# NethermindEth/starkpack-winterfell

Hardware: AMD Instinct MI355X
Metric: trace-LDE + Merkle-commit field-ops/s (wall-clock ms in ms_per_step), 2^20x8 f64 trace blowup=8 (higher is better)
Workload: dtype u64 (Goldilocks, Montgomery form) + u32 (BLAKE3)

## Files before the change

### include/wf_lde.h

```cpp
#ifndef WF_LDE_H
#define WF_LDE_H

#include <stddef.h>
#include <stdint.h>

#ifdef __cplusplus
extern "C" {
#endif

typedef struct wf_ctx wf_ctx;

enum wf_field { WF_FIELD_F64 = 1, WF_FIELD_F128 = 2 };
enum wf_hasher {
    WF_HASH_BLAKE3 = 0,
    WF_HASH_SHA3_256 = 1,
    WF_HASH_RP64_256 = 16,
    WF_HASH_RPJIVE64_256 = 18,
    WF_HASH_GRIFFINJIVE64_256 = 20
};

enum wf_status {
    WF_OK = 0,
    WF_ERR_FIELD = -10,
    WF_ERR_EXTENSION = -11,
// ... 18 lines not shown
    uint32_t log2_blowup;
    uint32_t n_cols;
    uint32_t n_traces;
    uint32_t digest_bytes;
    uint32_t hasher;
    uint8_t domain_offset[16];
} wf_params;


int wf_ctx_create(int device, wf_ctx **out);
void wf_ctx_destroy(wf_ctx *ctx);
int wf_ctx_release_cached(wf_ctx *ctx);
int wf_ctx_set_digest_bytes(wf_ctx *ctx, uint32_t digest_bytes);
int wf_ctx_set_hasher(wf_ctx *ctx, uint32_t hasher);
int wf_plan_digits(uint32_t field, uint32_t log2_n, uint32_t n_segments, uint32_t digits_out[4]);
const char *wf_last_error(void);
int wf_device_count(void);
int wf_ctx_synchronize(wf_ctx *ctx);
void *wf_ctx_stream(wf_ctx *ctx);

int wf_ctx_profile_enable(wf_ctx *ctx, int on);
int wf_ctx_profile_read(wf_ctx *ctx, int max_entries, const char **names, float *ms);

int wf_params_check(const wf_params *p, int is_constraint);

size_t wf_elem_bytes(uint32_t field);
size_t wf_row_width(const wf_params *p);
size_t wf_column_bytes(const wf_params *p);
size_t wf_lde_bytes(const wf_params *p);
size_t wf_digests_bytes(const wf_params *p);
// ... 214 lines not shown
```

### starkpack-winterfell_amd/capi.py

```python
from __future__ import annotations

import ctypes as C
import os
import weakref

import numpy as np

from .build import lib_path

F64, F128 = 1, 2
BLAKE3, SHA3_256, RP64_256, RPJIVE64_256, GRIFFINJIVE64_256 = 0, 1, 16, 18, 20
ELEM_WORDS = {F64: 1, F128: 2}

SYMBOLS = [
    "wf_ctx_create", "wf_ctx_destroy", "wf_last_error", "wf_device_count", "wf_ctx_synchronize", "wf_ctx_stream",
    "wf_ctx_release_cached", "wf_ctx_set_digest_bytes", "wf_ctx_set_hasher", "wf_plan_digits", "wf_commitment_query", "wf_ctx_profile_enable", "wf_ctx_profile_read", "wf_params_check", "wf_elem_bytes", "wf_row_width", "wf_column_bytes", "wf_lde_bytes", "wf_digests_bytes",
    "wf_trace_commit", "wf_constraint_commit", "wf_trace_commit_dev", "wf_constraint_commit_dev",
    "wf_trace_commit_shard_dev", "wf_merkle_build_dev", "wf_trace_commit_resident", "wf_trace_commit_resident_async", "wf_commitment_wait", "wf_constraint_commit_resident", "wf_commitment_destroy", "wf_commitment_root",
    "wf_commitment_info", "wf_commitment_read_rows", "wf_commitment_read_lde", "wf_commitment_read_lde_strided", "wf_deep_compose", "wf_commitment_evaluate_polys_at_points", "wf_constraint_commit_from_evaluations", "wf_constraint_commit_from_tables", "wf_commitment_query_many", "wf_commitment_prove", "wf_commitment_prove_batch",
    "wf_evaluate_columns_at", "wf_commitment_evaluate_polys_at", "wf_fri_layer_commit", "wf_fri_apply_drp", "wf_fri_layer_commit_dev", "wf_fri_apply_drp_dev",
    "wf_fri_prover_create", "wf_fri_prover_destroy", "wf_fri_num_layers", "wf_fri_prover_begin", "wf_fri_prover_begin_dev", "wf_fri_prover_begin_poly",
    "wf_fri_prover_commit_layer", "wf_fri_prover_fold", "wf_fri_prover_set_remainder", "wf_fri_prover_num_layers",
    "wf_fri_prover_layer", "wf_fri_prover_reset", "wf_fri_fold_positions",
    "wf_fft_evaluate_poly", "wf_fft_evaluate_poly_with_offset", "wf_fft_interpolate_poly",
    "wf_fft_interpolate_poly_with_offset", "wf_evaluate_polys_over", "wf_hash_rows", "wf_merkle_build", "wf_grind_seeds",
    "wf_comm_unique_id", "wf_comm_create", "wf_comm_create_with_transport", "wf_comm_destroy", "wf_comm_rank",
    "wf_comm_world", "wf_comm_rccl_version", "wf_comm_rccl_path", "wf_comm_stream_wait", "wf_comm_all_gather", "wf_comm_all_gather_roots", "wf_comm_barrier",
    "wf_comm_max_f64", "wf_comm_gather_f64", "wf_comm_info", "wf_shard_proofs", "wf_shard_cosets", "wf_shard_route", "wf_comm_all_gather_leaf_shards",
    "wf_trace_commit_sharded_dev", "wf_trace_commit_sharded_resident", "wf_sharded_commitment_destroy",
    "wf_sharded_commitment_root", "wf_sharded_commitment_query", "wf_sharded_commitment_polys",
    "wf_constraint_evaluate", "wf_evaluations_info", "wf_evaluations_read", "wf_evaluations_destroy",
    "wf_constraint_commit_from_device_tables",
]


class WfError(RuntimeError):
    def __init__(self, code: int, msg: str):
        super().__init__(f"wf_lde error {code}: {msg}")
        self.code = code


class Params(C.Structure):
    _fields_ = [
        ("field", C.c_uint32), ("ext_degree", C.c_uint32), ("log2_trace_len", C.c_uint32),
        ("log2_blowup", C.c_uint32), ("n_cols", C.c_uint32), ("n_traces", C.c_uint32),
        ("digest_bytes", C.c_uint32), ("hasher", C.c_uint32), ("domain_offset", C.c_uint8 * 16),
    ]
# ... 167 lines not shown
        L.wf_fri_prover_reset.argtypes = [vp]
        L.wf_fri_fold_positions.argtypes = [vp, sz, sz, u32, vp, C.POINTER(sz)]
        L.wf_fft_evaluate_poly.argtypes = [vp, u32, u32, vp, sz]
        L.wf_fft_interpolate_poly.argtypes = [vp, u32, u32, vp, sz]
        L.wf_fft_interpolate_poly_with_offset.argtypes = [vp, u32, u32, vp, sz, vp]
        L.wf_fft_evaluate_poly_with_offset.argtypes = [vp, u32, u32, vp, sz, vp, sz, vp]
        L.wf_evaluate_polys_over.argtypes = [vp, PP, vp, vp]
        L.wf_hash_rows.argtypes = [vp, u32, vp, sz, sz, vp]
        L.wf_merkle_build.argtypes = [vp, vp, sz, vp]
        L.wf_grind_seeds.argtypes = [vp, vp, sz, u32, C.c_uint64, C.c_uint64, vp, vp, vp]
        L.wf_device_count.argtypes = []
        L.wf_ctx_release_cached.argtypes = [vp]
        L.wf_ctx_set_digest_bytes.argtypes = [vp, u32]
        L.wf_ctx_set_hasher.argtypes = [vp, u32]
        L.wf_plan_digits.argtypes = [u32, u32, u32, C.POINTER(u32)]
        L.wf_commitment_query.argtypes = [vp, vp, sz, vp, vp, vp, sz, vp, C.POINTER(sz), C.POINTER(sz), C.POINTER(u32)]
        pu32, pu64 = C.POINTER(u32), C.POINTER(C.c_uint64)
        L.wf_comm_unique_id.argtypes = [vp]
        L.wf_comm_create.argtypes = [vp, vp, i32, i32, C.POINTER(vp)]
        L.wf_comm_create_with_transport.argtypes = [vp, C.POINTER(Transport), i32, i32, C.POINTER(vp)]
        L.wf_comm_destroy.argtypes = [vp]
        L.wf_comm_destroy.restype = None
        L.wf_comm_rank.argtypes = [vp]
        L.wf_comm_world.argtypes = [vp]
        L.wf_comm_rccl_version.argtypes = []
        L.wf_trace_commit_resident_async.argtypes = [vp, PP, vp, C.POINTER(vp)]
        L.wf_commitment_wait.argtypes = [vp]
        L.wf_comm_rccl_path.argtypes = []
        L.wf_comm_rccl_path.restype = C.c_char_p
        L.wf_comm_stream_wait.argtypes = [vp, vp]
# ... 573 lines not shown
        vecs, k = [], 0
        for i in range(q.n_vectors):
            vecs.append([bytes(nodes[k + j]) for j in range(int(counts[i]))])
            k += int(counts[i])
        out.append((rows, ([bytes(x) for x in leaves[:len(pos)]], vecs, int(q.depth))))
    return out


def plan_digits(field: int, log2_n: int, n_segments: int = 1):
    out = (C.c_uint32 * 4)()
    n = load().wf_plan_digits(field, log2_n, n_segments, out)
    _check(n if n < 0 else 0)
    return [int(out[i]) for i in range(n)]


def fri_num_layers(folding: int, blowup: int, remainder_max_degree: int, domain_size: int) -> int:
    return int(load().wf_fri_num_layers(folding, blowup, remainder_max_degree, domain_size))


def fri_fold_positions(positions, source_domain_size: int, folding: int) -> np.ndarray:
    pos = np.ascontiguousarray(positions, dtype=np.uint64)
    out = np.empty(max(1, len(pos)), dtype=np.uint64)
    n_out = C.c_size_t()
    _check(load().wf_fri_fold_positions(_p(pos), len(pos), source_domain_size, folding, _p(out), C.byref(n_out)))
    return out[:n_out.value].copy()


class FriProver:

    def __init__(self, ctx: "Context", field, ext, folding, blowup, remainder_max_degree, offset: int):
# ... 61 lines not shown
```

### starkpack-winterfell_amd/csrc/context.hip

```cpp
#include "wf_internal.hpp"

#include <atomic>

#include "field.hpp"
#include "hasher_table.hpp"

using namespace wf;

static thread_local char g_err[512] = "";

std::atomic<uint64_t> g_fail_epoch{0};
uint64_t fail_epoch() { return g_fail_epoch.load(std::memory_order_relaxed); }

int fail(int code, const char *fmt, ...) {
    g_fail_epoch.fetch_add(1, std::memory_order_relaxed);
    va_list ap;
    va_start(ap, fmt);
    vsnprintf(g_err, sizeof(g_err), fmt, ap);
    va_end(ap);
    return code;
}

const char *last_error_text() { return g_err; }

// ... 12 lines not shown
    t.persistent_always = getenv("WF_EXP_PERSISTENT_ALWAYS") != nullptr;
    t.no_persistent = getenv("WF_EXP_NO_PERSISTENT") != nullptr;
    if (const char *e = getenv("WF_EXP_MERKLE_L2_MIN")) {
        const int v = atoi(e);
        if (v >= 10 && v <= 30) t.merkle_l2_min = (uint32_t)v;
    }
    t.no_pipeline = getenv("WF_EXP_NO_PIPELINE") != nullptr;
    t.no_tail_pack = getenv("WF_EXP_NO_TAIL_PACK") != nullptr;
    t.no_coset_inner = getenv("WF_EXP_NO_COSET_INNER") != nullptr;
    t.no_gtab = getenv("WF_EXP_NO_GTAB") != nullptr;
    t.no_staged_chunks = getenv("WF_EXP_NO_STAGED_CHUNKS") != nullptr;
    t.no_gtab1 = getenv("WF_EXP_NO_GTAB1") != nullptr;
    t.no_ftab = getenv("WF_EXP_NO_FTAB") != nullptr;
    t.no_gtab1_wide = getenv("WF_EXP_NO_GTAB1_WIDE") != nullptr;
    t.gtab1_f64 = getenv("WF_EXP_GTAB1_F64") != nullptr;
    if (const char *e = getenv("WF_EXP_WIDE_TI")) {
        const int v = atoi(e);
        if (v == 1 || v == 2 || v == 4 || v == 8) t.wide_ti = (uint32_t)v;
    }
    if (const char *e = getenv("WF_EXP_PIPELINE_MIN_BYTES")) {
        const long long v = atoll(e);
        if (v >= 0 && v <= (1ll << 40)) t.pipeline_min_bytes = (size_t)v;
    }
    if (const char *e = getenv("WF_EXP_FAIL_AFTER_SEGMENT")) {
        const int v = atoi(e);
        if (v >= 0 && v < 4096) t.fail_after_segment = v;
    }
    if (const char *e = getenv("WF_EXP_GRIND_WINDOW_LOG2")) {
        const int v = atoi(e);
        if (v >= 2 && v <= 30) t.grind_window_log2 = (uint32_t)v;
// ... 403 lines not shown
```

### starkpack-winterfell_amd/csrc/path.hip

```cpp
#include "wf_internal.hpp"

#include "kernels.hpp"
#include "keccak_dev.hpp"
#include "keccak_kernels.hpp"
#include "merkle_plan.hpp"
#include "rescue_kernels.hpp"
#include "hasher_dispatch.hpp"
#include "seg_kernels.hpp"
#include "col_kernels.hpp"
#include "fri_kernels.hpp"
#include "tables.hpp"

using namespace wf;

#if defined(WF_EXPERIMENTS) && defined(WF_EXP_STAMPS)
static unsigned long long *g_exp_stamps = nullptr;
static unsigned long long *exp_stamps_buffer() {
    if (!g_exp_stamps && hipMalloc(&g_exp_stamps, 4096 * 8 * 8) == hipSuccess) (void)hipMemset(g_exp_stamps, 0, 4096 * 8 * 8);
    return g_exp_stamps;
}
extern "C" int wf_exp_stamps_read(unsigned long long *out, int clear) {
    if (!g_exp_stamps) return -1;
    if (hipMemcpy(out, g_exp_stamps, 4096 * 8 * 8, hipMemcpyDeviceToHost) != hipSuccess) return -2;
    if (clear) (void)hipMemset(g_exp_stamps, 0, 4096 * 8 * 8);
// ... 188 lines not shown
    T *out;
    uint32_t logN, n_seg, n_cosets;
    bool rows_out;
    void *leaves = nullptr;
    uint32_t hash_epr = 0;
    uint32_t digest_words = 8;
    bool *fused = nullptr;
    const TableSet *pre;
    const T *fin_tab = nullptr;
    bool pad_traces = false;
    bool pad_in_kernel = false;
    uint32_t base_cols, total_base_cols, coset0;
    uint64_t row_width, trace_lde_elems;
    uint32_t seg0 = 0, seg_cnt = 0;
    int phase = 0;
};

template <class F>
static int run_seg_transform(wf_ctx *ctx, hipStream_t st, const SegDesc<F> &d) {
    typedef typename F::T T;
    const bool inverse = !d.rows_out;
    TableSet *tw;
    int rc = root_tables<F>(ctx, d.logN, inverse, &tw);
    if (rc) return rc;
    const Plan plan = seg_plan<F>(d.logN, d.n_seg, ctx->tune.max_digit, ctx->tune.full_tiles);
    const uint64_t N = (uint64_t)1 << d.logN;

    SegArgs<F> a;
    memset(&a, 0, sizeof(a));
    a.logN = d.logN;
    a.n_seg = d.n_seg;
    a.n_cosets = d.n_cosets;
    a.tw = as_pow2l<F>(*tw);
    if (d.pre) {
        a.pre = as_pow2l<F>(*d.pre);
        a.pre_lo_stride = d.pre->lo_stride;
        a.pre_hi_stride = d.pre->hi_stride;
    }
    a.base_cols = d.base_cols;
    a.total_base_cols = d.total_base_cols;
    a.store_cols = d.pad_in_kernel ? d.n_seg * SegCfg<F>::S : d.base_cols;
// ... 520 lines not shown
            rc = run_merkle(ctx, st, d_leaves, Nrows, d_nodes, p->hasher, p->digest_bytes);
            if (rc) return rc;
        }
    }
    prof_mark(ctx, st, "between_calls");
    return 0;
}

template <class F>
static int trace_commit_dev(wf_ctx *ctx, const wf_params *p, const void *d_trace, void *d_polys, void *d_lde,
                            void *d_leaves, void *d_nodes, hipStream_t st, hipEvent_t input_read = nullptr) {
    PathBufs<F> b;
    int rc = path_buffers<F>(ctx, p, b);
    if (rc) return rc;
    const uint64_t R = (uint64_t)1 << p->log2_trace_len;
    rc = run_xpose<F>(ctx, st, true, d_trace, b.segA, R, p->ext_degree, b.total_base_cols, b.n_seg);
    if (rc) return rc;
    if (input_read) HIP_TRY(hipEventRecord(input_read, st));
    SegDesc<F> d;
    memset(&d, 0, sizeof(d));
    d.in = b.segA;
    d.work = b.segA;
    d.out = b.segB;
    d.logN = p->log2_trace_len;
    d.n_seg = b.n_seg;
    d.n_cosets = 1;
    d.rows_out = false;
    rc = run_seg_transform<F>(ctx, st, d);
    if (rc) return rc;
    rc = run_xpose<F>(ctx, st, false, b.segB, d_polys, R, p->ext_degree, b.total_base_cols, b.n_seg);
    if (rc) return rc;
    return evaluate_and_commit<F>(ctx, st, p, b, d_lde, d_leaves, d_nodes);
}

template <class F>
static int trace_commit_pipelined_impl(wf_ctx *ctx, const wf_params *p, const void *const *cols_in, void *d_stage, void *d_polys,
                                       void *d_lde, void *d_leaves, void *d_nodes, hipStream_t st, void *const *polys_out) {
    typedef typename F::T T;
    constexpr uint32_t S = SegCfg<F>::S;
    PathBufs<F> b;
    int rc = path_buffers<F>(ctx, p, b);
    if (rc) return rc;
// ... 2 lines not shown
    if (!ctx->copy_stream) HIP_TRY(hipStreamCreateWithFlags(&ctx->copy_stream, hipStreamNonBlocking));
    while (ctx->seg_events.size() < (size_t)b.n_seg + 1) {
        hipEvent_t e;
        HIP_TRY(hipEventCreateWithFlags(&e, hipEventDisableTiming));
        ctx->seg_events.push_back(e);
    }
    HIP_TRY(hipEventRecord(ctx->seg_events[b.n_seg], st));
    HIP_TRY(hipStreamWaitEvent(ctx->copy_stream, ctx->seg_events[b.n_seg], 0));
    for (uint32_t g = 0; g < b.n_seg; g++) {
        if (ctx->tune.fail_after_segment >= 0 && (int)g == ctx->tune.fail_after_segment)
            return fail(WF_ERR_HIP, "injected failure after %u uploaded segment(s) (WF_EXP_FAIL_AFTER_SEGMENT)", g);
        for (size_t i = (size_t)g * S; i < std::min<size_t>(TC, (size_t)(g + 1) * S); i++)
            HIP_TRY(hipMemcpyAsync((char *)d_stage + i * colb, cols_in[i], colb, hipMemcpyHostToDevice, ctx->copy_stream));
        HIP_TRY(hipEventRecord(ctx->seg_events[g], ctx->copy_stream));
        HIP_TRY(hipStreamWaitEvent(st, ctx->seg_events[g], 0));
        rc = run_xpose<F>(ctx, st, true, d_stage, b.segA, R, 1, b.total_base_cols, b.n_seg, g, 1);
        if (rc) return rc;
        SegDesc<F> d;
        memset(&d, 0, sizeof(d));
        d.in = b.segA + (size_t)g * R * S;
        d.work = (T *)d.in;
        d.out = b.segB + (size_t)g * R * S;
        d.logN = p->log2_trace_len;
        d.n_seg = 1;
        d.n_cosets = 1;
        d.rows_out = false;
        if ((rc = run_seg_transform<F>(ctx, st, d))) return rc;
        if ((rc = evaluate_and_commit<F>(ctx, st, p, b, d_lde, d_leaves, d_nodes, 0, 0, false, 1, g, 1))) return rc;
    }
    if ((rc = run_xpose<F>(ctx, st, false, b.segB, d_polys, R, 1, b.total_base_cols, b.n_seg))) return rc;
    if (polys_out) HIP_TRY(hipEventRecord(ctx->seg_events[b.n_seg], st));
    if ((rc = evaluate_and_commit<F>(ctx, st, p, b, d_lde, d_leaves, d_nodes, 0, 0, false, 2))) return rc;
    if (polys_out) {
        HIP_TRY(hipStreamWaitEvent(ctx->copy_stream, ctx->seg_events[b.n_seg], 0));
        if ((rc = download_columns(ctx, polys_out, d_polys, TC, colb, ctx->copy_stream))) return rc;
        HIP_TRY(hipStreamSynchronize(ctx->copy_stream));
    }
    return 0;
}

template <class F>
// ... 45 lines not shown
    return p->field == WF_FIELD_F64 ? packed_shape<F64>(1, base, base, 1u << p->log2_blowup, &cpr, &lg)
                                    : packed_shape<F128>(1, base, base, 1u << p->log2_blowup, &cpr, &lg);
}

extern "C" {

int wf_plan_digits(uint32_t field, uint32_t log2_n, uint32_t n_segments, uint32_t digits_out[4]) {
    if (!digits_out) return fail(WF_ERR_ARG, "digits_out is null");
    if (field != WF_FIELD_F64 && field != WF_FIELD_F128) return fail(WF_ERR_FIELD, "unknown field id %u", field);
    if (log2_n < 1 || log2_n > 40) return fail(WF_ERR_TRACE_LENGTH, "transform size out of range");
    const Plan p = field == WF_FIELD_F64 ? seg_plan<F64>(log2_n, n_segments) : seg_plan<F128>(log2_n, n_segments);
    for (int i = 0; i < 4; i++) digits_out[i] = i < p.n_pass ? p.dig[i] : 0;
    return p.n_pass;
}


int wf_trace_commit_dev(wf_ctx *ctx, const wf_params *p, const void *d_trace, void *d_polys, void *d_lde,
                        void *d_leaves, void *d_nodes, void *stream) {
    if (!ctx) return fail(WF_ERR_ARG, "ctx is null");
    int rc = check_params(p, false);
    if (rc) return rc;
    if (!d_trace || !d_polys || !d_lde) return fail(WF_ERR_ARG, "null device buffer");
    HIP_TRY(hipSetDevice(ctx->device));
    hipStream_t st = stream ? (hipStream_t)stream : ctx->stream;
    WF_ENTER(ctx, st);
    if (p->field == WF_FIELD_F64) return trace_commit_dev<F64>(ctx, p, d_trace, d_polys, d_lde, d_leaves, d_nodes, st);
    return trace_commit_dev<F128>(ctx, p, d_trace, d_polys, d_lde, d_leaves, d_nodes, st);
}

int wf_constraint_commit_dev(wf_ctx *ctx, const wf_params *p, const void *d_polys, void *d_lde, void *d_leaves,
// ... 481 lines not shown
```

### starkpack-winterfell_amd/csrc/seg_kernels.hpp

```cpp
#pragma once

#include <hip/hip_runtime.h>
#include <stdint.h>

#include "field.hpp"
#include "kernels.hpp"

#ifndef WF_EXPERIMENTS
#undef WF_EXP_SKIP_LOAD
#undef WF_EXP_SKIP_NTT
#undef WF_EXP_SKIP_STORE
#undef WF_EXP_LOCAL_STORE
#undef WF_EXP_STAMPS
#endif

namespace wf {

template <class F>
struct SegCfg {
    static constexpr uint32_t S = 64 / F::BYTES;
    static constexpr uint32_t HP = S / 2;
    static constexpr bool RADIX16 = F::BYTES == 8;
    static constexpr bool RADIX8 = F::BYTES == 16;
    static constexpr uint32_t LOAD_BATCH = F::BYTES == 8 ? 8 : 4;
// ... 25 lines not shown
template <>
__device__ __forceinline__ Pair<uint64_t> pair_from<F64>(const uint4 &qa, const uint4 &) {
    Pair<uint64_t> v;
    v.a = ((uint64_t)qa.y << 32) | qa.x;
    v.b = ((uint64_t)qa.w << 32) | qa.z;
    return v;
}
template <>
__device__ __forceinline__ Pair<U128> pair_from<F128>(const uint4 &qa, const uint4 &qb) {
    Pair<U128> v;
    v.a = U128{((uint64_t)qa.y << 32) | qa.x, ((uint64_t)qa.w << 32) | qa.z};
    v.b = U128{((uint64_t)qb.y << 32) | qb.x, ((uint64_t)qb.w << 32) | qb.z};
    return v;
}

enum : int { SEG_OUT_SEG = 0, SEG_OUT_ROWS = 1 };

template <int LOGD>
__device__ __forceinline__ uint32_t tile_threads() {
    return LOGD ? (1u << (LOGD ? LOGD - 1 : 0)) : blockDim.x;
}
#define WF_TILE_BOUNDS(LOGD, GENERIC) __launch_bounds__((LOGD) ? (1 << ((LOGD) ? (LOGD) - 1 : 0)) : (GENERIC), (LOGD) ? 4 : 1)

__device__ __forceinline__ uint64_t xcd_group_index(uint64_t b, uint64_t total) {
    if ((total & 63) != 0) return b;
    const uint64_t xcd = b & 7, seq = b >> 3;
    return (((seq >> 3) << 3) + xcd) * 8 + (seq & 7);
}

__device__ __forceinline__ uint64_t coset_inner_split(uint64_t bid, uint32_t lc, uint32_t &c) {
    const uint64_t hi = bid >> 6;
// ... 33 lines not shown
    uint32_t tail_pad;
    uint32_t seg_stride;
    uint32_t coset0;
    uint32_t rows_per_k;
    uint32_t cpr_log, lg_log;
    uint64_t row_width;
    uint64_t trace_lde_elems;
    uint32_t *leaves;
    uint32_t hash_epr;
    uint32_t digest_words;
    uint32_t *chunk_cvs;
    uint32_t n_chunks;
    uint32_t *tile_counters;
    const T *src_tail;
    uint32_t tail_cols;
#ifdef WF_EXP_STAMPS
    unsigned long long *stamps;
#endif
};

#if defined(WF_EXPERIMENTS) && defined(WF_EXP_R8_NO_SPLIT)
constexpr uint32_t R8_SPLIT = 0;
#else
constexpr uint32_t R8_SPLIT = 4;
#endif
__host__ __device__ constexpr uint32_t radix8_rounds(uint32_t logD) {
    return (R8_SPLIT == 4 && logD >= 4 && logD % 3 == 1) ? logD / 3 - 1 : logD / 3;
}

template <class F>
// ... 431 lines not shown
    if (logD >= 2) w4 = twd[D >> 2];
    while (cur > 0) {
        if (cur >= 2) {
            seg_round4<F, DIR, false, LANES>(x, twd, w4, logD, cur, nthr, threadIdx.x);
            cur -= 2;
        } else {
            seg_round2<F, LANES>(x, logD, nthr, threadIdx.x);
            cur = 0;
        }
        __syncthreads();
    }
}

template <class F, int EVAL, bool PACKED = false, int LOGD = 0>
__global__ void WF_TILE_BOUNDS(LOGD, 1024) k_seg_strided(SegArgs<F> a) {
    typedef typename F::T T;
    if (LOGD) a.logD = LOGD;
    const uint32_t NT = tile_threads<LOGD>();
    typedef Pair<T> P2;
    constexpr uint32_t S = SegCfg<F>::S, HP = SegCfg<F>::HP;
    constexpr uint32_t hp_shift = HP == 4 ? 2 : 1;
    extern __shared__ __attribute__((aligned(16))) unsigned char smem_raw[];
    const uint32_t D = 1u << a.logD;
    T *x = reinterpret_cast<T *>(smem_raw);
    T *twd = x + (size_t)D * S;
    constexpr bool ONE_TABLE = F::BYTES == 16;
    T *aux = ONE_TABLE ? twd : twd + D;

    uint64_t bid = xcd_group_index(blockIdx.x, gridDim.x);
    const uint32_t logI = ilog2_pow2(a.I), logO = ilog2_pow2(a.O);
// ... 170 lines not shown
#undef WF_FILL_ITEM
    }
    if (!direct || scale_in) __syncthreads();
    if (ONE_TABLE) {
        if (threadIdx.x < D) twd[kq[0]] = unpark<F>(twk0);
        if (threadIdx.x + NT < D) twd[kq[1]] = unpark<F>(twk1);
        __syncthreads();
    } else {
#pragma unroll
        for (uint32_t q = 0; q < 2; q++) {
            const uint32_t k = threadIdx.x + q * NT;
            if (k < D) aux[k] = fo[q];
        }
    }
#ifndef WF_EXP_SKIP_NTT
    seg_lds_ntt<F, EVAL ? 1 : -1, (LOGD ? (1u << LOGD) : 0u)>(x, twd, a.logD, NT, direct ? vr : nullptr, direct);
#else
    if (direct && has16) {
#pragma unroll
        for (uint32_t q = 0; q < 16; q++) x[(q * m16 + j16) * S + l16] = vr[q];
    }
    __syncthreads();
#endif
    if (ONE_TABLE) {
        if (threadIdx.x < D) aux[threadIdx.x] = unpark<F>(fok0);
        if (threadIdx.x + NT < D) aux[threadIdx.x + NT] = unpark<F>(fok1);
        __syncthreads();
    }

    T start_a = F::one(), start_b = F::one();
    if (PACKED && a.pre_on) {
// ... 2 lines not shown
    }
    const uint32_t pstride = NT >> hp_shift, pos0 = threadIdx.x >> hp_shift;
    if (pos0 >= D) return;
    const uint32_t k0 = seg_digit_reverse<F>(pos0, a.logD);
    T *dst_lane = dst + row0 * S + lane_a;
    const uint32_t k_shift = logI + (S == 8 ? 3 : 2);
    for (uint32_t pj = 0; pj < D; pj += pstride) {
        const uint32_t k = k0 | seg_digit_reverse<F>(pj, a.logD);
        P2 v = *reinterpret_cast<P2 *>(x + (pos0 + pj) * S + lane_a);
        const T f = aux[k];
        v.a = F::mul(v.a, f);
        v.b = F::mul(v.b, f);
        if (PACKED && a.pre_on) {
            v.a = F::mul(v.a, start_a);
            v.b = F::mul(v.b, start_b);
        }
#ifdef WF_EXP_SKIP_STORE
        if (*reinterpret_cast<const uint32_t *>(&v.a) == a.logN + 77777u)
#endif
        store_pair(dst_lane + ((uint64_t)k << k_shift), v);
    }
}

template <class F, int EVAL, int TI, int GTAB = 0, int LOGD = 0>
__global__ void __launch_bounds__(1024) k_seg_strided_wide(SegArgs<F> a) {
    if (LOGD) a.logD = LOGD;
    static_assert(SegCfg<F>::RADIX16 && TI >= 2 && (TI & (TI - 1)) == 0, "f64 tiles of 2, 4 or 8 inner positions");
    typedef typename F::T T;
    typedef Pair<T> P2;
    constexpr uint32_t S = SegCfg<F>::S, LANES = TI * S, HPW = LANES / 2;
// ... 177 lines not shown
        for (uint32_t pos = psub; pos < D; pos += pstep) {
            const uint64_t k = rev_o + ((uint64_t)seg_digit_reverse<F>(pos, a.logD) << out_shift);
            const uint64_t off = (uint64_t)(uint32_t)k * k_stride;
            const T v0 = d0 && in0 ? x[pos * S + (b0 - lo)] : F::zero();
            const T v1 = d1 && in1 ? x[pos * S + (b1 - lo)] : F::zero();
            if (in0 && in1)
                store_pair(row + off, Pair<T>{v0, v1});
            else if (in0)
                row[off] = v0;
            else
                row[off + 1] = v1;
        }
    }
}

template <class F, int OUT, bool PACKED = false, int LOGD = 0>
__global__ void WF_TILE_BOUNDS(LOGD, 1024) k_seg_last(SegArgs<F> a) {
    typedef typename F::T T;
    const uint32_t logD_ = LOGD ? (uint32_t)LOGD : a.logD;
    const uint32_t NT = tile_threads<LOGD>();
    typedef Pair<T> P2;
    constexpr uint32_t S = SegCfg<F>::S, HP = SegCfg<F>::HP;
    constexpr uint32_t hp_shift = HP == 4 ? 2 : 1;
    extern __shared__ __attribute__((aligned(16))) unsigned char smem_raw[];
    const uint32_t D = 1u << logD_;
    T *x = reinterpret_cast<T *>(smem_raw);
    T *twd = x + (size_t)D * S;
    T *aux = twd;

    uint64_t bid = xcd_group_index(blockIdx.x, gridDim.x);
    const uint32_t logO = ilog2_pow2(a.O);
    const uint32_t b32 = (uint32_t)bid;
    const uint32_t q32 = b32 / a.n_cosets, c = b32 - q32 * a.n_cosets;
    const uint64_t o = q32 & (uint32_t)(a.O - 1);
    const uint32_t g = q32 >> logO;
    const uint64_t seg_elems = ((uint64_t)1 << a.logN) * S;
    const T *src = a.src + (a.src_shared ? (uint64_t)g : (uint64_t)c * a.n_seg + g) * seg_elems + (o << logD_) * S;

    uint64_t rev_o = 0;
    {
        uint32_t bits = 0;
        for (uint32_t q = 0; q < a.n_prev; q++) bits += a.prev_log[q];
        uint32_t hi = bits, sh = 0;
        for (uint32_t q = 0; q < a.n_prev; q++) {
            hi -= a.prev_log[q];
            rev_o |= ((o >> hi) & (((uint64_t)1 << a.prev_log[q]) - 1)) << sh;
            sh += a.prev_log[q];
        }
    }

    Pow2L<F> pre = a.pre, pre_a = a.pre, pre_b = a.pre;
    const uint32_t lane_a = 2 * (threadIdx.x & (HP - 1)), lane_b = lane_a + 1;
// ... 32 lines not shown
    r0 = r1 = r2 = r3 = r4 = r5 = r6 = r7 = make_uint4(0, 0, 0, 0);
#ifdef WF_EXP_SKIP_LOAD
#define WF_ITEM_PTR(WK) reinterpret_cast<const uint4 *>(a.src + 2 * (uint64_t)((WK) & 63))
#else
#define WF_ITEM_PTR(WK) reinterpret_cast<const uint4 *>(src + 2 * (uint64_t)(WK))
#endif
#define WF_LOAD_ITEM(U, RA, RB)                            \
    do {                                                   \
        const uint32_t wk_ = threadIdx.x + (U) * step;     \
        if (wk_ < nitems) {                                \
            const uint4 *p_ = WF_ITEM_PTR(wk_);            \
            RA = p_[0];                                    \
            if (F::BYTES == 16) RB = p_[1];                \
        }                                                  \
    } while (0)
    if (from_regs) {
        if (F::BYTES == 8) {
            WF_LOAD_ITEM(0, r0, r0);
            WF_LOAD_ITEM(1, r1, r1);
            WF_LOAD_ITEM(2, r2, r2);
            WF_LOAD_ITEM(3, r3, r3);
            WF_LOAD_ITEM(4, r4, r4);
            WF_LOAD_ITEM(5, r5, r5);
            WF_LOAD_ITEM(6, r6, r6);
            WF_LOAD_ITEM(7, r7, r7);
        } else {
            WF_LOAD_ITEM(0, r0, r1);
            WF_LOAD_ITEM(1, r2, r3);
            WF_LOAD_ITEM(2, r4, r5);
            WF_LOAD_ITEM(3, r6, r7);
        }
    }
#undef WF_LOAD_ITEM
#undef WF_ITEM_PTR
#pragma unroll
    for (uint32_t q = 0; q < 2; q++) {
        if (threadIdx.x + q * NT < D) {
            if (scale_in)
                aux[kq[q]] = (!PACKED && a.fin_tab) ? fi_a[q] : F::mul(fi_a[q], fi_b[q]);
            else
                twd[kq[q]] = unpark<F>(q == 0 ? twk0 : twk1);
        }
    }
    __syncthreads();
    if (PACKED && a.pre_on) {
        for (uint32_t wk = threadIdx.x; wk < nitems; wk += NT) {
            P2 v;
            const uint32_t d = wk >> hp_shift;
            const uint32_t lgm = (1u << a.lg_log) - 1, cola = lane_a & lgm, colb = lane_b & lgm;
            const T *srow = src + (uint64_t)d * S;
            const T fa = pre_a.get(d);
            const T fb = a.lg_log ? fa : pre_b.get(d);
            v.a = act_a ? F::mul(srow[cola], fa) : F::zero();
            v.b = act_b ? F::mul(srow[colb], fb) : F::zero();
            *reinterpret_cast<P2 *>(x + 2 * wk) = v;
        }
    } else {
#define WF_FILL_ITEM(U, RA, RB)                                \
    do {                                                       \
        const uint32_t wk_ = threadIdx.x + (U) * step;         \
// ... 770 lines not shown
```

### starkpack-winterfell_amd/csrc/tables.hpp

```cpp
#pragma once

#include "wf_internal.hpp"

#include "pow2l.hpp"

using namespace wf;

static int table_upload(wf_ctx *ctx, void **dst, const void *src, size_t bytes) {
    *dst = nullptr;
    hipError_t e = dev_malloc(ctx, dst, bytes);
    if (e != hipSuccess) return fail(WF_ERR_HIP, "table allocation of %zu bytes failed: %s", bytes, hipGetErrorString(e));
    e = hipMemcpy(*dst, src, bytes, hipMemcpyHostToDevice);
    if (e != hipSuccess) {
        (void)hipFree(*dst);
        *dst = nullptr;
        return fail(WF_ERR_HIP, "table upload failed: %s", hipGetErrorString(e));
    }
    return 0;
}

template <class F>
static int upload_pow2l(wf_ctx *ctx, const std::vector<typename F::T> &bases, uint32_t logN, TableSet &ts) {
    typedef typename F::T T;
    const uint32_t s = (logN + 1) / 2;
// ... 182 lines not shown
                tab[i * D + k] = acc;
                acc = F::mul(acc, step);
            }
            step = F::mul(step, base);
        }
        TableSet ts;
        const int rcu = table_upload(ctx, &ts.lo, tab.data(), tab.size() * sizeof(T));
        if (rcu) return rcu;
        it = ctx->tables.emplace(key, ts).first;
    }
    *out = (const typename F::T *)it->second.lo;
    return 0;
}

template <class F>
static typename F::T offset_elem(const wf_params *p, uint64_t &lo, uint64_t &hi) {
    u128 off;
    memcpy(&off, p->domain_offset, 16);
    lo = (uint64_t)off;
    hi = (uint64_t)(off >> 64);
    return F::from_u128_canonical(off);
}
```

### starkpack-winterfell_amd/csrc/wf_internal.hpp

```cpp
#pragma once

#include "../../include/wf_lde.h"

#include <hip/hip_runtime.h>

#include <algorithm>
#include <atomic>
#include <cstdarg>
#include <cstdio>
#include <cstring>
#include <map>
#include <mutex>
#include <set>
#include <string>
#include <thread>
#include <tuple>
#include <type_traits>
#include <vector>

int fail(int code, const char *fmt, ...) __attribute__((format(printf, 2, 3)));
const char *last_error_text();
uint64_t fail_epoch();

#define HIP_TRY(expr)                                                                              \
// ... 19 lines not shown
    bool no_specialized = false;
    bool no_fused_hash = false;
    bool no_chunked = false;
    bool persistent_always = false;
    bool no_persistent = false;
    uint32_t merkle_l2_min = 18;
    bool no_pipeline = false;
    size_t pipeline_min_bytes = (size_t)1 << 20;
    bool no_tail_pack = false;
    bool no_coset_inner = false;
    bool no_gtab1_wide = false;
    bool no_ftab = false;
    bool no_gtab1 = false;
    bool gtab1_f64 = false;
    bool no_staged_chunks = false;
    bool no_gtab = false;
    uint32_t wide_ti = 0;
    int fail_after_segment = -1;
    uint32_t grind_window_log2 = 0;
    uint32_t grind_window_cap_log2 = 0;
};
wf_tuning tuning_from_env();

struct wf_ctx {
    int device = 0;
    int num_cus = 256;
    wf_tuning tune;
    uint32_t digest_bytes = 32;
    uint32_t hasher = WF_HASH_BLAKE3;
    DevBuf pack_tmp;
// ... 190 lines not shown
```

Before: 1949 billion.

## Interpolate trace directly from column layout, skipping the input transpose

After: 1973 billion (median of 6 runs). +1.3%, better.

```diff
diff --git a/include/wf_lde.h b/include/wf_lde.h
--- a/include/wf_lde.h
+++ b/include/wf_lde.h
@@ -56,6 +56,7 @@
 int wf_ctx_set_digest_bytes(wf_ctx *ctx, uint32_t digest_bytes);
 int wf_ctx_set_hasher(wf_ctx *ctx, uint32_t hasher);
 int wf_plan_digits(uint32_t field, uint32_t log2_n, uint32_t n_segments, uint32_t digits_out[4]);
+int wf_interp_lane_factors(uint32_t log2_n, uint32_t log2_d, uint32_t log2_i, uint64_t *out);
 const char *wf_last_error(void);
 int wf_device_count(void);
 int wf_ctx_synchronize(wf_ctx *ctx);
diff --git a/starkpack-winterfell_amd/capi.py b/starkpack-winterfell_amd/capi.py
--- a/starkpack-winterfell_amd/capi.py
+++ b/starkpack-winterfell_amd/capi.py
@@ -30,7 +30,7 @@
     "wf_trace_commit_sharded_dev", "wf_trace_commit_sharded_resident", "wf_sharded_commitment_destroy",
     "wf_sharded_commitment_root", "wf_sharded_commitment_query", "wf_sharded_commitment_polys",
     "wf_constraint_evaluate", "wf_evaluations_info", "wf_evaluations_read", "wf_evaluations_destroy",
-    "wf_constraint_commit_from_device_tables",
+    "wf_constraint_commit_from_device_tables", "wf_interp_lane_factors",
 ]
 
 
@@ -228,6 +228,8 @@
         L.wf_ctx_set_digest_bytes.argtypes = [vp, u32]
         L.wf_ctx_set_hasher.argtypes = [vp, u32]
         L.wf_plan_digits.argtypes = [u32, u32, u32, C.POINTER(u32)]
+        if hasattr(L, "wf_interp_lane_factors"):
+            L.wf_interp_lane_factors.argtypes = [u32, u32, u32, vp]
         L.wf_commitment_query.argtypes = [vp, vp, sz, vp, vp, vp, sz, vp, C.POINTER(sz), C.POINTER(sz), C.POINTER(u32)]
         pu32, pu64 = C.POINTER(u32), C.POINTER(C.c_uint64)
         L.wf_comm_unique_id.argtypes = [vp]
@@ -831,6 +833,12 @@
     return [int(out[i]) for i in range(n)]
 
 
+def interp_lane_factors(log2_n: int, log2_d: int, log2_i: int) -> np.ndarray:
+    out = np.empty((1 << log2_d, 8), dtype=np.uint64)
+    _check(load().wf_interp_lane_factors(log2_n, log2_d, log2_i, _p(out)))
+    return out
+
+
 def fri_num_layers(folding: int, blowup: int, remainder_max_degree: int, domain_size: int) -> int:
     return int(load().wf_fri_num_layers(folding, blowup, remainder_max_degree, domain_size))
 
diff --git a/starkpack-winterfell_amd/csrc/context.hip b/starkpack-winterfell_amd/csrc/context.hip
--- a/starkpack-winterfell_amd/csrc/context.hip
+++ b/starkpack-winterfell_amd/csrc/context.hip
@@ -50,6 +50,7 @@
     t.no_ftab = getenv("WF_EXP_NO_FTAB") != nullptr;
     t.no_gtab1_wide = getenv("WF_EXP_NO_GTAB1_WIDE") != nullptr;
     t.gtab1_f64 = getenv("WF_EXP_GTAB1_F64") != nullptr;
+    t.no_colsrc = getenv("WF_EXP_NO_COLSRC") != nullptr;
     if (const char *e = getenv("WF_EXP_WIDE_TI")) {
         const int v = atoi(e);
         if (v == 1 || v == 2 || v == 4 || v == 8) t.wide_ti = (uint32_t)v;
diff --git a/starkpack-winterfell_amd/csrc/path.hip b/starkpack-winterfell_amd/csrc/path.hip
--- a/starkpack-winterfell_amd/csrc/path.hip
+++ b/starkpack-winterfell_amd/csrc/path.hip
@@ -226,7 +226,90 @@
     uint64_t row_width, trace_lde_elems;
     uint32_t seg0 = 0, seg_cnt = 0;
     int phase = 0;
+    const T *cols_in = nullptr;
+    hipEvent_t cols_read = nullptr;
 };
+
+template <class F>
+static bool interp_from_cols_ok(const wf_ctx *ctx, uint32_t logN, uint32_t n_seg, uint32_t ext_degree, const void *cols) {
+    if (F::BYTES != 8 || ext_degree != 1 || ctx->tune.no_colsrc || ((uintptr_t)cols & 15) != 0) return false;
+    const Plan plan = seg_plan<F>(logN, n_seg, ctx->tune.max_digit, ctx->tune.full_tiles);
+    return plan.n_pass <= 2 && plan.dig[plan.n_pass - 1] >= 3;
+}
+
+template <class F>
+static int run_interp_from_cols(wf_ctx *ctx, hipStream_t st, const SegDesc<F> &d, const Plan &plan) {
+    if constexpr (F::BYTES != 8) {
+        return fail(WF_ERR_ARG, "internal: column-source interpolation is f64 only");
+    } else {
+        const bool two = plan.n_pass == 2;
+        SegArgs<F> a;
+        memset(&a, 0, sizeof(a));
+        a.n_cosets = 1;
+        a.total_base_cols = d.total_base_cols;
+        a.scale = f_inv<F>(F::from_u128_canonical((u128)1 << d.logN));
+        TableSet *tw;
+        int rc;
+        uint32_t threads;
+        size_t lds;
+        if (two) {
+            const uint32_t logD = plan.dig[0], logI = plan.dig[1];
+            if ((rc = root_tables<F>(ctx, d.logN - 3, true, &tw))) return rc;
+            a.tw = as_pow2l<F>(*tw);
+            a.logN = d.logN - 3;
+            a.logD = logD;
+            a.O = 1;
+            a.I = (uint64_t)1 << (logI - 3);
+            a.n_seg = a.seg_stride = d.total_base_cols;
+            if ((rc = digit_table<F>(ctx, logD, true, &a.digit_tw))) return rc;
+            if ((rc = lane_factor_table<F>(ctx, d.logN, logD, logI, true, &a.lane_tab))) return rc;
+            a.src = d.cols_in;
+            a.dst = d.work;
+            a.scale_on = 1;
+            if ((rc = seg_launch_dims<F>(logD, threads, lds, false))) return rc;
+            const uint64_t grid = (uint64_t)d.total_base_cols * a.I;
+            if (grid > 0x7FFFFFFFull) return fail(WF_ERR_ARG, "problem too large for one launch (%llu groups)", (unsigned long long)grid);
+            const void *kern = (const void *)k_seg_strided<F, SEG_INTERP_COLS>;
+            if (threads * 2 == (1u << logD) && !ctx->tune.no_specialized) {
+                if (logD == 10) kern = (const void *)k_seg_strided<F, SEG_INTERP_COLS, false, 10>;
+                if (logD == 9) kern = (const void *)k_seg_strided<F, SEG_INTERP_COLS, false, 9>;
+            }
+            if (lds > 64 * 1024) HIP_TRY(hipFuncSetAttribute(kern, hipFuncAttributeMaxDynamicSharedMemorySize, 160 * 1024));
+            prof_mark(ctx, st, "interpolate.strided_pass");
+            void *kargs[] = {&a};
+            HIP_TRY(hipLaunchKernel(kern, dim3((uint32_t)grid), dim3(threads), kargs, lds, st));
+            if (d.cols_read) HIP_TRY(hipEventRecord(d.cols_read, st));
+            a.lane_tab = nullptr;
+        }
+        if ((rc = root_tables<F>(ctx, d.logN, true, &tw))) return rc;
+        a.tw = as_pow2l<F>(*tw);
+        a.logN = d.logN;
+        a.logD = plan.dig[plan.n_pass - 1];
+        a.O = two ? (uint64_t)1 << plan.dig[0] : 1;
+        a.I = 1;
+        a.n_seg = a.seg_stride = d.n_seg;
+        a.n_prev = plan.n_pass - 1;
+        a.prev_log[0] = two ? plan.dig[0] : 0;
+        if ((rc = digit_table<F>(ctx, a.logD, true, &a.digit_tw))) return rc;
+        a.src = two ? d.work : d.cols_in;
+        a.dst = d.out;
+        a.scale_on = two ? 0 : 1;
+        if ((rc = seg_launch_dims<F>(a.logD, threads, lds, true))) return rc;
+        const uint64_t grid = (uint64_t)d.n_seg * a.O;
+        if (grid > 0x7FFFFFFFull) return fail(WF_ERR_ARG, "problem too large for one launch (%llu groups)", (unsigned long long)grid);
+        const void *kern = (const void *)k_seg_last<F, SEG_OUT_SEG_COLS>;
+        if (threads * 2 == (1u << a.logD) && !ctx->tune.no_specialized) {
+            if (a.logD == 10) kern = (const void *)k_seg_last<F, SEG_OUT_SEG_COLS, false, 10>;
+            if (a.logD == 9) kern = (const void *)k_seg_last<F, SEG_OUT_SEG_COLS, false, 9>;
+        }
+        if (lds > 64 * 1024) HIP_TRY(hipFuncSetAttribute(kern, hipFuncAttributeMaxDynamicSharedMemorySize, 160 * 1024));
+        prof_mark(ctx, st, "interpolate.last_pass");
+        void *kargs[] = {&a};
+        HIP_TRY(hipLaunchKernel(kern, dim3((uint32_t)grid), dim3(threads), kargs, lds, st));
+        if (!two && d.cols_read) HIP_TRY(hipEventRecord(d.cols_read, st));
+        return 0;
+    }
+}
 
 template <class F>
 static int run_seg_transform(wf_ctx *ctx, hipStream_t st, const SegDesc<F> &d) {
@@ -237,6 +320,10 @@
     if (rc) return rc;
     const Plan plan = seg_plan<F>(d.logN, d.n_seg, ctx->tune.max_digit, ctx->tune.full_tiles);
     const uint64_t N = (uint64_t)1 << d.logN;
+    if (d.cols_in) {
+        if (d.rows_out || d.phase != 0 || d.seg0 != 0 || plan.n_pass > 2) return fail(WF_ERR_ARG, "internal: column-source transform of a shape it does not serve");
+        return run_interp_from_cols<F>(ctx, st, d, plan);
+    }
 
     SegArgs<F> a;
     memset(&a, 0, sizeof(a));
@@ -787,9 +874,6 @@
     int rc = path_buffers<F>(ctx, p, b);
     if (rc) return rc;
     const uint64_t R = (uint64_t)1 << p->log2_trace_len;
-    rc = run_xpose<F>(ctx, st, true, d_trace, b.segA, R, p->ext_degree, b.total_base_cols, b.n_seg);
-    if (rc) return rc;
-    if (input_read) HIP_TRY(hipEventRecord(input_read, st));
     SegDesc<F> d;
     memset(&d, 0, sizeof(d));
     d.in = b.segA;
@@ -799,6 +883,15 @@
     d.n_seg = b.n_seg;
     d.n_cosets = 1;
     d.rows_out = false;
+    if (interp_from_cols_ok<F>(ctx, p->log2_trace_len, b.n_seg, p->ext_degree, d_trace)) {
+        d.cols_in = (const typename F::T *)d_trace;
+        d.total_base_cols = b.total_base_cols;
+        d.cols_read = input_read;
+    } else {
+        rc = run_xpose<F>(ctx, st, true, d_trace, b.segA, R, p->ext_degree, b.total_base_cols, b.n_seg);
+        if (rc) return rc;
+        if (input_read) HIP_TRY(hipEventRecord(input_read, st));
+    }
     rc = run_seg_transform<F>(ctx, st, d);
     if (rc) return rc;
     rc = run_xpose<F>(ctx, st, false, b.segB, d_polys, R, p->ext_degree, b.total_base_cols, b.n_seg);
@@ -831,8 +924,6 @@
             HIP_TRY(hipMemcpyAsync((char *)d_stage + i * colb, cols_in[i], colb, hipMemcpyHostToDevice, ctx->copy_stream));
         HIP_TRY(hipEventRecord(ctx->seg_events[g], ctx->copy_stream));
         HIP_TRY(hipStreamWaitEvent(st, ctx->seg_events[g], 0));
-        rc = run_xpose<F>(ctx, st, true, d_stage, b.segA, R, 1, b.total_base_cols, b.n_seg, g, 1);
-        if (rc) return rc;
         SegDesc<F> d;
         memset(&d, 0, sizeof(d));
         d.in = b.segA + (size_t)g * R * S;
@@ -842,6 +933,14 @@
         d.n_seg = 1;
         d.n_cosets = 1;
         d.rows_out = false;
+        const T *seg_cols = (const T *)d_stage + (size_t)g * S * R;
+        if (interp_from_cols_ok<F>(ctx, p->log2_trace_len, 1, 1, seg_cols)) {
+            d.cols_in = seg_cols;
+            d.total_base_cols = (uint32_t)(std::min<size_t>(TC, (size_t)(g + 1) * S) - (size_t)g * S);
+        } else {
+            rc = run_xpose<F>(ctx, st, true, d_stage, b.segA, R, 1, b.total_base_cols, b.n_seg, g, 1);
+            if (rc) return rc;
+        }
         if ((rc = run_seg_transform<F>(ctx, st, d))) return rc;
         if ((rc = evaluate_and_commit<F>(ctx, st, p, b, d_lde, d_leaves, d_nodes, 0, 0, false, 1, g, 1))) return rc;
     }
@@ -917,6 +1016,14 @@
     return p.n_pass;
 }
 
+int wf_interp_lane_factors(uint32_t log2_n, uint32_t log2_d, uint32_t log2_i, uint64_t *out) {
+    if (!out) return fail(WF_ERR_ARG, "out is null");
+    if (log2_n < 1 || log2_n > 32 || log2_d > 11 || log2_d + log2_i > log2_n)
+        return fail(WF_ERR_ARG, "lane factors of a pass [2^%u tiles, 2^%u inner positions] of 2^%u rows", log2_d, log2_i, log2_n);
+    const std::vector<uint64_t> tab = lane_factors_host<F64>(log2_n, log2_d, log2_i, true);
+    memcpy(out, tab.data(), tab.size() * sizeof(uint64_t));
+    return 0;
+}
 
 int wf_trace_commit_dev(wf_ctx *ctx, const wf_params *p, const void *d_trace, void *d_polys, void *d_lde,
                         void *d_leaves, void *d_nodes, void *stream) {
diff --git a/starkpack-winterfell_amd/csrc/seg_kernels.hpp b/starkpack-winterfell_amd/csrc/seg_kernels.hpp
--- a/starkpack-winterfell_amd/csrc/seg_kernels.hpp
+++ b/starkpack-winterfell_amd/csrc/seg_kernels.hpp
@@ -63,7 +63,8 @@
     return v;
 }
 
-enum : int { SEG_OUT_SEG = 0, SEG_OUT_ROWS = 1 };
+enum : int { SEG_OUT_SEG = 0, SEG_OUT_ROWS = 1, SEG_OUT_SEG_COLS = 2 };
+enum : int { SEG_INTERP = 0, SEG_EVAL = 1, SEG_INTERP_COLS = 2 };
 
 template <int LOGD>
 __device__ __forceinline__ uint32_t tile_threads() {
@@ -127,6 +128,7 @@
     uint32_t *tile_counters;
     const T *src_tail;
     uint32_t tail_cols;
+    const T *lane_tab;
 #ifdef WF_EXP_STAMPS
     unsigned long long *stamps;
 #endif
@@ -588,6 +590,8 @@
 
 template <class F, int EVAL, bool PACKED = false, int LOGD = 0>
 __global__ void WF_TILE_BOUNDS(LOGD, 1024) k_seg_strided(SegArgs<F> a) {
+    constexpr bool LANETAB = EVAL == SEG_INTERP_COLS;
+    static_assert(!LANETAB || (!PACKED && F::BYTES == 8), "the column view is an f64 interpolation");
     typedef typename F::T T;
     if (LOGD) a.logD = LOGD;
     const uint32_t NT = tile_threads<LOGD>();
@@ -788,7 +792,7 @@
         }
     }
 #ifndef WF_EXP_SKIP_NTT
-    seg_lds_ntt<F, EVAL ? 1 : -1, (LOGD ? (1u << LOGD) : 0u)>(x, twd, a.logD, NT, direct ? vr : nullptr, direct);
+    seg_lds_ntt<F, EVAL == 1 ? 1 : -1, (LOGD ? (1u << LOGD) : 0u)>(x, twd, a.logD, NT, direct ? vr : nullptr, direct);
 #else
     if (direct && has16) {
 #pragma unroll
@@ -821,6 +825,11 @@
         if (PACKED && a.pre_on) {
             v.a = F::mul(v.a, start_a);
             v.b = F::mul(v.b, start_b);
+        }
+        if constexpr (LANETAB) {
+            const P2 e = *reinterpret_cast<const P2 *>(a.lane_tab + k * S + lane_a);
+            v.a = F::mul(v.a, e.a);
+            v.b = F::mul(v.b, e.b);
         }
 #ifdef WF_EXP_SKIP_STORE
         if (*reinterpret_cast<const uint32_t *>(&v.a) == a.logN + 77777u)
@@ -1028,8 +1037,11 @@
     }
 }
 
-template <class F, int OUT, bool PACKED = false, int LOGD = 0>
+template <class F, int OUT_, bool PACKED = false, int LOGD = 0>
 __global__ void WF_TILE_BOUNDS(LOGD, 1024) k_seg_last(SegArgs<F> a) {
+    constexpr bool COLSRC = OUT_ == SEG_OUT_SEG_COLS;
+    constexpr int OUT = COLSRC ? (int)SEG_OUT_SEG : OUT_;
+    static_assert(!COLSRC || (!PACKED && F::BYTES == 8), "column-source tiles: the f64 interpolation");
     typedef typename F::T T;
     const uint32_t logD_ = LOGD ? (uint32_t)LOGD : a.logD;
     const uint32_t NT = tile_threads<LOGD>();
@@ -1049,7 +1061,7 @@
     const uint64_t o = q32 & (uint32_t)(a.O - 1);
     const uint32_t g = q32 >> logO;
     const uint64_t seg_elems = ((uint64_t)1 << a.logN) * S;
-    const T *src = a.src + (a.src_shared ? (uint64_t)g : (uint64_t)c * a.n_seg + g) * seg_elems + (o << logD_) * S;
+    const T *src = a.src + (a.src_shared ? (uint64_t)g : (uint64_t)c * a.n_seg + g) * seg_elems + (o << logD_) * (COLSRC ? 1 : S);
 
     uint64_t rev_o = 0;
     {
@@ -1112,7 +1124,25 @@
             if (F::BYTES == 16) RB = p_[1];                \
         }                                                  \
     } while (0)
-    if (from_regs) {
+    if constexpr (COLSRC) {
+        const uint32_t cj = threadIdx.x & (S - 1);
+        if (g * S + cj < a.total_base_cols) {
+            const uint4 *pc = reinterpret_cast<const uint4 *>(src + ((uint64_t)cj << a.logN)) + (threadIdx.x >> 3);
+#define WF_LOAD_COL(U, RA)                                                      \
+    do {                                                                        \
+        if (threadIdx.x + (U) * step < nitems) RA = pc[(U) * (step >> 3)];      \
+    } while (0)
+            WF_LOAD_COL(0, r0);
+            WF_LOAD_COL(1, r1);
+            WF_LOAD_COL(2, r2);
+            WF_LOAD_COL(3, r3);
+            WF_LOAD_COL(4, r4);
+            WF_LOAD_COL(5, r5);
+            WF_LOAD_COL(6, r6);
+            WF_LOAD_COL(7, r7);
+#undef WF_LOAD_COL
+        }
+    } else if (from_regs) {
         if (F::BYTES == 8) {
             WF_LOAD_ITEM(0, r0, r0);
             WF_LOAD_ITEM(1, r1, r1);
@@ -1141,7 +1171,27 @@
         }
     }
     __syncthreads();
-    if (PACKED && a.pre_on) {
+    if constexpr (COLSRC) {
+#define WF_FILL_COL(U, RA)                                              \
+    do {                                                                \
+        const uint32_t wk_ = threadIdx.x + (U) * step;                  \
+        if (wk_ < nitems) {                                             \
+            const P2 v_ = pair_from<F>(RA, RA);                         \
+            T *px_ = x + (wk_ >> 3) * (2 * S) + (wk_ & (S - 1));        \
+            px_[0] = v_.a;                                              \
+            px_[S] = v_.b;                                              \
+        }                                                               \
+    } while (0)
+        WF_FILL_COL(0, r0);
+        WF_FILL_COL(1, r1);
+        WF_FILL_COL(2, r2);
+        WF_FILL_COL(3, r3);
+        WF_FILL_COL(4, r4);
+        WF_FILL_COL(5, r5);
+        WF_FILL_COL(6, r6);
+        WF_FILL_COL(7, r7);
+#undef WF_FILL_COL
+    } else if (PACKED && a.pre_on) {
         for (uint32_t wk = threadIdx.x; wk < nitems; wk += NT) {
             P2 v;
             const uint32_t d = wk >> hp_shift;
diff --git a/starkpack-winterfell_amd/csrc/tables.hpp b/starkpack-winterfell_amd/csrc/tables.hpp
--- a/starkpack-winterfell_amd/csrc/tables.hpp
+++ b/starkpack-winterfell_amd/csrc/tables.hpp
@@ -220,6 +220,42 @@
 }
 
 template <class F>
+static std::vector<typename F::T> lane_factors_host(uint32_t logN, uint32_t logD, uint32_t logI, bool inverse) {
+    typedef typename F::T T;
+    constexpr uint32_t S = 64 / F::BYTES;
+    T w = f_root_of_unity<F>(logN ? logN : 1);
+    if (inverse) w = f_inv<F>(w);
+    const T base = f_pow<F>(w, (u128)1 << (logN - logD - logI));
+    const size_t D = (size_t)1 << logD;
+    std::vector<T> tab(D * S);
+    T step = F::one();
+    for (size_t k = 0; k < D; k++) {
+        T acc = F::one();
+        for (uint32_t t = 0; t < S; t++) {
+            tab[k * S + t] = acc;
+            acc = F::mul(acc, step);
+        }
+        step = F::mul(step, base);
+    }
+    return tab;
+}
+
+template <class F>
+static int lane_factor_table(wf_ctx *ctx, uint32_t logN, uint32_t logD, uint32_t logI, bool inverse, const typename F::T **out) {
+    auto key = std::make_tuple((int)F::FIELD_ID, (int)logN, inverse ? 10 : 9, (int)(logD | (logI << 8)), (uint64_t)0, (uint64_t)0);
+    auto it = ctx->tables.find(key);
+    if (it == ctx->tables.end()) {
+        const std::vector<typename F::T> tab = lane_factors_host<F>(logN, logD, logI, inverse);
+        TableSet ts;
+        const int rcu = table_upload(ctx, &ts.lo, tab.data(), tab.size() * sizeof(typename F::T));
+        if (rcu) return rcu;
+        it = ctx->tables.emplace(key, ts).first;
+    }
+    *out = (const typename F::T *)it->second.lo;
+    return 0;
+}
+
+template <class F>
 static typename F::T offset_elem(const wf_params *p, uint64_t &lo, uint64_t &hi) {
     u128 off;
     memcpy(&off, p->domain_offset, 16);
diff --git a/starkpack-winterfell_amd/csrc/wf_internal.hpp b/starkpack-winterfell_amd/csrc/wf_internal.hpp
--- a/starkpack-winterfell_amd/csrc/wf_internal.hpp
+++ b/starkpack-winterfell_amd/csrc/wf_internal.hpp
@@ -57,6 +57,7 @@
     bool no_gtab1 = false;
     bool gtab1_f64 = false;
     bool no_staged_chunks = false;
+    bool no_colsrc = false;
     bool no_gtab = false;
     uint32_t wide_ti = 0;
     int fail_after_segment = -1;
```
